# hila-chefer/Transformer-Explainability

Measured on NVIDIA H100. Metric: explanations_per_sec, higher is better.
Workload: dtype f32

## Files before the change

### transformer_explainability_b200/csrc/te_tc_wgmma.cu

```cuda
#include <cuda.h>
#include <cuda_bf16.h>
#include <cuda_fp16.h>
#include <cuda_runtime.h>
#include <string.h>
#include <algorithm>
#include <string>
#include <type_traits>
#include <utility>

#include "te_gemm_tc.h"
#include "te_wgmma.cuh"

namespace {

constexpr int BM = 128, NTHREADS = 256;

__device__ __forceinline__ uint32_t smem_u32(const void* p) { return (uint32_t)__cvta_generic_to_shared(p); }
__device__ __forceinline__ void fence_proxy_async() { asm volatile("fence.proxy.async.shared::cta;" ::: "memory"); }
__device__ __forceinline__ void wg_fence() { asm volatile("wgmma.fence.sync.aligned;" ::: "memory"); }
__device__ __forceinline__ void wg_commit() { asm volatile("wgmma.commit_group.sync.aligned;" ::: "memory"); }
__device__ __forceinline__ void wg_wait0() { asm volatile("wgmma.wait_group.sync.aligned 0;" ::: "memory"); }
__device__ __forceinline__ void wg_wait1() { asm volatile("wgmma.wait_group.sync.aligned 1;" ::: "memory"); }

__device__ __forceinline__ void mbar_init(uint32_t bar, uint32_t count) {
// ... 157 lines not shown
        for (int u = 0; u < 4; ++u) {
            const int k = 4 * c + u;
            e[u] = *reinterpret_cast<const float*>(box + k * 128 + (((m >> 2) ^ (k & 7)) << 4));
        }
        f(r, c, make_float4(e[0], e[1], e[2], e[3]));
    }
}
template <bool SP>
__device__ __forceinline__ auto put_tf32(uint8_t* hi, uint8_t* lo) {
    return [=](int r, int c, float4 v) {
        if (SP) st4(hi, r, c, tf32x4(v));
        else st_split(hi, lo, r, c, v);
    };
}
template <bool SP>
__device__ __forceinline__ void fix_tf32(uint8_t* hi, uint8_t* lo, int r0, int n, int t, int nt) {
    if (SP) map_rows(hi, r0, n, t, nt, [](float4 v) { return tf32x4(v); });
    else split_rows(hi, lo, r0, n, t, nt);
}

__device__ __forceinline__ int frag_row(int tid, int j) { return 64 * (tid >> 7) + 16 * ((tid >> 5) & 3) + ((tid & 31) >> 2) + 8 * ((j >> 1) & 1); }
__device__ __forceinline__ int frag_col(int tid, int j) { return 8 * (j >> 2) + 2 * (tid & 3) + (j & 1); }

struct TmaArgs {
    CUtensorMap map[4];
    int mtiles, ntiles, nz;
};
enum { FIX_NONE = 0, FIX_A = 1, FIX_AB = 2 };
constexpr int NTHREADS_TMA = 384, SMEM_MAX = 227 * 1024;
__host__ __device__ constexpr int tma_stages(int bytes) { return (SMEM_MAX - 1024 - 128) / bytes < 8 ? (SMEM_MAX - 1024 - 128) / bytes : 8; }

template <class P, int NA, int NR, int NT, int NTR>
__device__ __forceinline__ void fold(const P& p, float (&acc)[NA][NR], float (&tot)[NT][NTR], int m0, int ch, int z, int tid) {
    const float s0 = p.chunk_scale(m0 + frag_row(tid, 0), ch, z), s1 = p.chunk_scale(m0 + frag_row(tid, 2), ch, z);
#pragma unroll
    for (int a = 0; a < NA; ++a)
#pragma unroll
        for (int j = 0; j < NR; ++j) tot[a][j] = fmaf(acc[a][j], ((j >> 1) & 1) ? s1 : s0, tot[a][j]);
}
template <int NA, int NR>
__device__ __forceinline__ void zero(float (&v)[NA][NR]) {
#pragma unroll
    for (int a = 0; a < NA; ++a)
#pragma unroll
        for (int j = 0; j < NR; ++j) v[a][j] = 0.f;
}

template <class P>
__device__ __forceinline__ void reg_tile(const P& p, uint8_t* smem, int col_fast) {
    constexpr int NR = P::BN / 2;
    constexpr int NA = P::PRODS::NACC;
    constexpr int STAGE = P::L::BYTES;
    constexpr int NT = P::CHUNK ? NA : 1, NTR = P::CHUNK ? NR : 1;
// ... 1 lines not shown
    const int m0 = (col_fast ? blockIdx.y : blockIdx.x) * BM, n0 = (col_fast ? blockIdx.x : blockIdx.y) * P::BN;
    const int z = blockIdx.z;
    float acc[NA][NR];
    float tot[NT][NTR];
    zero(acc);
    zero(tot);

    const int kb = p.kblocks();
    p.load(smem, 0, m0, n0, z, tid);
    fence_proxy_async();
    __syncthreads();
    for (int it = 0; it < kb; ++it) {
        const bool fresh = P::CHUNK ? (it % P::CHUNK == 0) : (it == 0);
        wg_fence();
        issue<P>(smem_u32(smem + (it & 1) * STAGE), wg, acc, fresh ? 0u : 1u);
        wg_commit();
        if (it + 1 < kb) p.load(smem + ((it + 1) & 1) * STAGE, it + 1, m0, n0, z, tid);
        wg_wait0();
        if constexpr (P::CHUNK > 0)
            if ((it + 1) % P::CHUNK == 0 || it + 1 == kb) fold(p, acc, tot, m0, it / P::CHUNK, z, tid);
        fence_proxy_async();
        __syncthreads();
    }
    if constexpr (P::CHUNK > 0) p.epilogue(tot, m0, n0, z, tid);
    else p.epilogue(acc, m0, n0, z, tid);
}

template <class P>
__device__ __forceinline__ void tma_tiles(const P& p, const TmaArgs& ta, uint8_t* smem) {
    using L = typename P::L;
    constexpr int NR = P::BN / 2;
    constexpr int NA = P::PRODS::NACC;
    constexpr int STAGE = L::BYTES, S = tma_stages(STAGE);
    constexpr int NT = P::CHUNK ? NA : 1, NTR = P::CHUNK ? NR : 1;
    static_assert(S >= 2, "a TMA problem needs two stages");
    __shared__ __align__(8) uint64_t bars[2 * S];
    const int tid = threadIdx.x, wg = tid >> 7;
    const uint32_t full0 = smem_u32(bars), empty0 = full0 + 8u * S, st0 = smem_u32(smem);
    if (tid == 0) {
        for (int s = 0; s < S; ++s) {
            mbar_init(full0 + 8u * s, 1);
            mbar_init(empty0 + 8u * s, 8);
        }
        asm volatile("fence.mbarrier_init.release.cluster;" ::: "memory");
    }
    __syncthreads();
    const int kb = p.kblocks(), per_z = ta.mtiles * ta.ntiles, ntiles = ta.nz * per_z;
    int stage = 0;
    uint32_t phase = 0;
    auto decode = [&](int t, int& m0, int& n0, int& z) {
        z = t / per_z;
        const int r = t - z * per_z;
        m0 = (r / ta.ntiles) * BM;
        n0 = (r % ta.ntiles) * P::BN;
    };

    if (wg == 2) {
        setmaxnreg_dec<40>();
        if (tid != 2 * 128) return;
        for (int t = blockIdx.x; t < ntiles; t += gridDim.x) {
            int m0, n0, z;
            decode(t, m0, n0, z);
            for (int it = 0; it < kb; ++it) {
                mbar_wait(empty0 + 8u * stage, phase ^ 1u);
                p.produce(ta, st0 + (uint32_t)stage * STAGE, full0 + 8u * stage, it, m0, n0, z);
                if (++stage == S) { stage = 0; phase ^= 1u; }
            }
        }
        return;
    }

    setmaxnreg_inc<232>();
    float acc[NA][NR];
    float tot[NT][NTR];
    auto release = [&](int s) {
        if ((tid & 31) == 0) mbar_arrive(empty0 + 8u * s);
    };
    for (int t = blockIdx.x; t < ntiles; t += gridDim.x) {
        int m0, n0, z;
        decode(t, m0, n0, z);
        zero(acc);
        zero(tot);
        int pend = -1;
        for (int it = 0; it < kb; ++it) {
            mbar_wait(full0 + 8u * stage, phase);
            const uint32_t st = st0 + (uint32_t)stage * STAGE;
            if constexpr (P::FIX != FIX_NONE) {
                p.fix(smem + (uint32_t)stage * STAGE, wg, tid);
                fence_proxy_async();
                if constexpr (P::FIX == FIX_A) bar_named(1 + wg, 128);
                else bar_named(3, 256);
            }
            const bool fresh = P::CHUNK ? (it % P::CHUNK == 0) : (it == 0);
            wg_fence();
            issue<P>(st, wg, acc, fresh ? 0u : 1u);
            wg_commit();
            const bool last = it + 1 == kb;
            if (last || (P::CHUNK ? (it + 1) % P::CHUNK == 0 : false)) {
                wg_wait0();
                if (pend >= 0) release(pend);
                release(stage);
                pend = -1;
                if constexpr (P::CHUNK > 0) fold(p, acc, tot, m0, it / P::CHUNK, z, tid);
            } else {
                wg_wait1();
                if (pend >= 0) release(pend);
                pend = stage;
            }
            if (++stage == S) { stage = 0; phase ^= 1u; }
        }
        if constexpr (P::CHUNK > 0) p.epilogue(tot, m0, n0, z, tid);
        else p.epilogue(acc, m0, n0, z, tid);
    }
}

template <class P>
__global__ void __launch_bounds__(P::TMA ? NTHREADS_TMA : NTHREADS, 1)
    wg_kernel(const P p, const __grid_constant__ TmaArgs ta, int col_fast) {
    extern __shared__ uint8_t smem_raw[];
    uint8_t* smem = smem_raw + ((1024u - (smem_u32(smem_raw) & 1023u)) & 1023u);
    if constexpr (P::TMA) tma_tiles(p, ta, smem);
    else reg_tile(p, smem, col_fast);
}

struct NoScale {
    __device__ __forceinline__ float chunk_scale(int, int, int) const { return 1.f; }
};

struct TmaTile {
    const void* base;
    long long rows, cols, ld;
    int box_rows;
    long long count = 0, cstride = 0;
};
template <class P>
// ... 1 lines not shown
    using L = typename P::L;
    constexpr int KE = P::FMT == OP_TF32 ? 32 : 64;
    mbar_expect_tx(bar, L::BYTES);
#pragma unroll
    for (int i = 0; i < L::NTA; ++i) tma_load(st + L::a(i), &ta.map[i], it * KE, m0, bar);
#pragma unroll
    for (int j = 0; j < L::NTB; ++j) tma_load(st + L::b(j), &ta.map[L::NTA + j], it * KE, n0, bar);
}
#define TE_PRODUCE_TILES(P)                                                                                      \
    static constexpr int NMAPS = L::NTA + L::NTB;                                                                \
    __device__ void produce(const TmaArgs& ta, uint32_t st, uint32_t bar, int it, int m0, int n0, int) const { \
        produce_tiles<P>(ta, st, bar, it, m0, n0);                                                               \
    }

enum { ZO_F32 = 0, ZO_BF16 = 1, ZO_F16S = 2 };
template <bool SINGLE, bool BF, int OUT>
struct ZsProb : NoScale {
    static constexpr int BN = 128, CHUNK = 0, FMT = BF ? OP_BF16 : OP_TF32;
    using PRODS = std::conditional_t<SINGLE, One, Prods<Pr<0, 0, 0>, Pr<0, 1, 1>>>;
    using L = Stage<PRODS, BN>;
    static constexpr bool COL_FAST = true;
    static constexpr bool TMA = SINGLE;
    static constexpr int FIX = SINGLE && !BF ? FIX_A : FIX_NONE;
    int M, N, K;
    const float* x; long long ldx;
    const void* xabs;
    const void* wa; const void* wb;
    const float* r; long long ldr; const float* y; long long ldy; const float* bias;
    void* out; long long ldo; float* hs;
    float sscale, zsign;

    __device__ int kblocks() const { return K / (BF ? 64 : 32); }
    __device__ void fix(uint8_t* st, int wg, int tid) const {
        map_rows(st + L::a(0), 64 * wg, 64, tid & 127, 128, [](float4 v) { return tf32x4(absx4(v)); });
    }
    TE_PRODUCE_TILES(ZsProb)
    TmaTile tile(int i) const {
        if (i == 0) return BF ? TmaTile{xabs, M, K, K, BM} : TmaTile{x, M, K, ldx, BM};
        return TmaTile{wa, N, K, K, BN};
    }
    __device__ void load(uint8_t* st, int kb, int m0, int n0, int, int tid) const {
        for_k32(BM, x, ldx, m0, M, kb * 32, K, tid, [&](int rr, int c, float4 v) {
            st4(st + L::a(0), rr, c, tf32x4(posx4(v)));
            st4(st + L::a(1), rr, c, tf32x4(negx4(v)));
        });
        for_k32(BN, (const float*)wa, K, n0, N, kb * 32, K, tid, [&](int rr, int c, float4 v) { st4(st + L::b(0), rr, c, v); });
        for_k32(BN, (const float*)wb, K, n0, N, kb * 32, K, tid, [&](int rr, int c, float4 v) { st4(st + L::b(1), rr, c, v); });
    }
    __device__ void epilogue(float (&acc)[1][BN / 2], int m0, int n0, int, int tid) const {
        float sv[BN / 2];
        float rmax[2] = {0.f, 0.f};
#pragma unroll
        for (int j = 0; j < BN / 2; j += 2) {
            const int row = m0 + frag_row(tid, j), col = n0 + frag_col(tid, j);
            float2 rr = make_float2(0.f, 0.f), z = make_float2(acc[0][j], acc[0][j + 1]);
            if (row < M) {
                rr = *reinterpret_cast<const float2*>(r + (long long)row * ldr + col);
                if (SINGLE) {
                    const float2 yy = *reinterpret_cast<const float2*>(y + (long long)row * ldy + col);
                    const float2 bb = bias ? *reinterpret_cast<const float2*>(bias + col) : make_float2(0.f, 0.f);
                    z.x = 0.5f * ((yy.x - bb.x) + zsign * z.x);
                    z.y = 0.5f * ((yy.y - bb.y) + zsign * z.y);
                    z = zsign > 0.f ? make_float2(fmaxf(z.x, 0.f), fmaxf(z.y, 0.f)) : make_float2(fminf(z.x, 0.f), fminf(z.y, 0.f));
                }
            }
            sv[j] = sscale * te_sd(rr.x, z.x);
            sv[j + 1] = sscale * te_sd(rr.y, z.y);
            if (OUT == ZO_F16S) rmax[(j >> 1) & 1] = fmaxf(rmax[(j >> 1) & 1], fmaxf(fabsf(sv[j]), fabsf(sv[j + 1])));
            if (row >= M) continue;
            if (OUT == ZO_F32) {
                *reinterpret_cast<float2*>((float*)out + (long long)row * ldo + col) = make_float2(to_tf32(sv[j]), to_tf32(sv[j + 1]));
            } else if (OUT == ZO_BF16) {
                *reinterpret_cast<__nv_bfloat162*>((__nv_bfloat16*)out + (long long)row * ldo + col) = __floats2bfloat162_rn(sv[j], sv[j + 1]);
            }
        }
        if (OUT == ZO_F16S) {
            float sc[2];
#pragma unroll
            for (int h = 0; h < 2; ++h) {
                float m = rmax[h];
                m = fmaxf(m, __shfl_xor_sync(0xffffffffu, m, 1));
                m = fmaxf(m, __shfl_xor_sync(0xffffffffu, m, 2));
                float si;
                te_f16_block_scale(m, sc[h], si);
                const int row = m0 + frag_row(tid, 2 * h);
                if ((tid & 3) == 0 && row < M) hs[(long long)row * (N / 128) + n0 / 128] = si;
            }
#pragma unroll
            for (int j = 0; j < BN / 2; j += 2) {
                const int row = m0 + frag_row(tid, j), col = n0 + frag_col(tid, j);
                const float s = sc[(j >> 1) & 1];
                if (row < M) *reinterpret_cast<__half2*>((__half*)out + (long long)row * N + col) = __floats2half2_rn(sv[j] * s, sv[j + 1] * s);
            }
        }
    }
};

template <int KIND>
struct ZrProb {
    static constexpr int BN = (KIND == 2) ? 64 : 128, CHUNK = (KIND == 2) ? 2 : 0;
    static constexpr int FMT = KIND == 0 ? OP_TF32 : KIND == 1 ? OP_BF16 : OP_F16;
    using PRODS = Prods<Pr<0, 0, 0>, Pr<1, 0, 1>>;
    using L = Stage<PRODS, BN>;
    static constexpr bool TMA = true;
    static constexpr int FIX = FIX_NONE;
    int M, N, K;
    const void* s; const void* wp; const void* wn;
    const float* rs; int rs_ld; const float* cp; const float* cn;
    const float* x; long long ldx; float* out; long long ldo;
    int accum;

    __device__ int kblocks() const { return K / (KIND ? 64 : 32); }
    TE_PRODUCE_TILES(ZrProb)
    __device__ float chunk_scale(int row, int ch, int) const { return (KIND == 2 && row < M) ? rs[(long long)row * rs_ld + ch] : 1.f; }
    TmaTile tile(int i) const { return i == 0 ? TmaTile{s, M, K, K, BM} : TmaTile{i == 1 ? wp : wn, N, K, K, BN}; }
    __device__ void epilogue(float (&acc)[2][BN / 2], int m0, int n0, int, int tid) const {
#pragma unroll
        for (int j = 0; j < BN / 2; j += 2) {
            const int row = m0 + frag_row(tid, j), col = n0 + frag_col(tid, j);
            if (row >= M) continue;
            const float2 xv = *reinterpret_cast<const float2*>(x + (long long)row * ldx + col);
            float2 ap = make_float2(acc[0][j], acc[0][j + 1]), an = make_float2(acc[1][j], acc[1][j + 1]);
            if (KIND == 2) {
                ap.x *= cp[col]; ap.y *= cp[col + 1];
                an.x *= cn[col]; an.y *= cn[col + 1];
            }
            float2* o = reinterpret_cast<float2*>(out + (long long)row * ldo + col);
            float2 v = make_float2(fmaxf(xv.x, 0.f) * ap.x + fminf(xv.x, 0.f) * an.x, fmaxf(xv.y, 0.f) * ap.y + fminf(xv.y, 0.f) * an.y);
            if (accum) {
                const float2 prev = *o;
                v = make_float2(prev.x + v.x, prev.y + v.y);
            }
            *o = v;
        }
    }
};

template <bool NEG>
struct LrpSProb : NoScale {
    static constexpr int BN = 128, CHUNK = 0, FMT = OP_TF32;
    using PRODS = One;
    using L = Stage<PRODS, BN>;
    static constexpr bool COL_FAST = true, TMA = false;
    int M, N, K;
    const float* x; long long ldx; const float* w;
    const float* r; long long ldr; float* out;
    float sscale;
    __device__ int kblocks() const { return K / 32; }
    __device__ void load(uint8_t* st, int kb, int m0, int n0, int, int tid) const {
        for_k32(BM, x, ldx, m0, M, kb * 32, K, tid, [&](int rr, int c, float4 v) { st4(st + L::a(0), rr, c, tf32x4(NEG ? negx4(v) : posx4(v))); });
        for_k32(BN, w, K, n0, N, kb * 32, K, tid, [&](int rr, int c, float4 v) { st4(st + L::b(0), rr, c, v); });
    }
    __device__ void epilogue(float (&acc)[1][BN / 2], int m0, int n0, int, int tid) const {
#pragma unroll
        for (int j = 0; j < BN / 2; j += 2) {
            const int row = m0 + frag_row(tid, j), col = n0 + frag_col(tid, j);
            if (row >= M) continue;
            const float2 rr = *reinterpret_cast<const float2*>(r + (long long)row * ldr + col);
            *reinterpret_cast<float2*>(out + (long long)row * N + col) =
                make_float2(to_tf32(sscale * te_sd(rr.x, acc[0][j])), to_tf32(sscale * te_sd(rr.y, acc[0][j + 1])));
        }
    }
};
template <bool NEG>
struct LrpRProb : NoScale {
    static constexpr int BN = 128, CHUNK = 0, FMT = OP_TF32;
    using PRODS = One;
    using L = Stage<PRODS, BN>;
    static constexpr bool TMA = true;
    static constexpr int FIX = FIX_NONE;
    int M, N, K;
    const float* s; const float* wt;
    const float* x; long long ldx; float* out; long long ldo;
    int accum;
    __device__ int kblocks() const { return K / 32; }
    TE_PRODUCE_TILES(LrpRProb)
    TmaTile tile(int i) const { return i == 0 ? TmaTile{s, M, K, K, BM} : TmaTile{wt, N, K, K, BN}; }
    __device__ void epilogue(float (&acc)[1][BN / 2], int m0, int n0, int, int tid) const {
#pragma unroll
        for (int j = 0; j < BN / 2; j += 2) {
            const int row = m0 + frag_row(tid, j), col = n0 + frag_col(tid, j);
            if (row >= M) continue;
            const float2 xv = *reinterpret_cast<const float2*>(x + (long long)row * ldx + col);
            float2* o = reinterpret_cast<float2*>(out + (long long)row * ldo + col);
            if (NEG) {
                const float2 prev = *o;
                *o = make_float2(prev.x + fminf(xv.x, 0.f) * acc[0][j], prev.y + fminf(xv.y, 0.f) * acc[0][j + 1]);
            } else if (accum) {
                const float2 prev = *o;
                *o = make_float2(prev.x + fmaxf(xv.x, 0.f) * acc[0][j], prev.y + fmaxf(xv.y, 0.f) * acc[0][j + 1]);
            } else {
                *o = make_float2(fmaxf(xv.x, 0.f) * acc[0][j], fmaxf(xv.y, 0.f) * acc[0][j + 1]);
            }
        }
    }
};

struct LinOut {
    int M, N;
    const float* bias; const float* E; long long lde;
    float* C; long long ldc; float* C2; long long ldc2;
};
template <int EPI, bool FAST_GRAD = false>
__device__ __forceinline__ void lin_store(const LinOut& o, int row, int col, float v0, float v1) {
    if (row >= o.M) return;
    float2 b = make_float2(0.f, 0.f);
    if ((EPI == TE_TC_EPI_BIAS || EPI == TE_TC_EPI_BIAS_GELU || EPI == TE_TC_EPI_BIAS_ADD) && o.bias)
        b = *reinterpret_cast<const float2*>(o.bias + col);
    float2 y = make_float2(v0 + b.x, v1 + b.y), y2 = make_float2(0.f, 0.f);
    if (EPI == TE_TC_EPI_BIAS_GELU) y2 = make_float2(te_gelu(y.x), te_gelu(y.y));
    if (EPI == TE_TC_EPI_BIAS_ADD || EPI == TE_TC_EPI_GELU_BWD) {
        const float2 e = *reinterpret_cast<const float2*>(o.E + (long long)row * o.lde + col);
        if (EPI == TE_TC_EPI_BIAS_ADD) y2 = make_float2(e.x + y.x, e.y + y.y);
        else if (FAST_GRAD) y = make_float2(v0 * te_gelu_grad_fast(e.x), v1 * te_gelu_grad_fast(e.y));
        else y = make_float2(v0 * te_gelu_grad(e.x), v1 * te_gelu_grad(e.y));
    }
    *reinterpret_cast<float2*>(o.C + (long long)row * o.ldc + col) = y;
    if (EPI == TE_TC_EPI_BIAS_GELU || EPI == TE_TC_EPI_BIAS_ADD) *reinterpret_cast<float2*>(o.C2 + (long long)row * o.ldc2 + col) = y2;
}

enum { LIN_3XTF32 = 0, LIN_TF32 = 1, LIN_F16X3 = 2, LIN_F16 = 3 };
struct LinArgs {
    int K, rs_ld;
    const void* a; const void* a_lo; long long lda;
    const void* b; const void* b_lo;
    const float* rs; const float* cs;
    LinOut o;
};
static_assert(sizeof(LinArgs) <= 128, "LinArgs: keep the kernel parameter within 128 bytes");
template <int EPI, int FORM>
struct LinProb : LinArgs {
    static constexpr bool F16 = FORM == LIN_F16X3 || FORM == LIN_F16, SPLIT = FORM == LIN_3XTF32 || FORM == LIN_F16X3;
    static constexpr int BN = 128, CHUNK = F16 ? 2 : SPLIT ? 4 : 0, FMT = F16 ? OP_F16 : OP_TF32;
    using PRODS = std::conditional_t<SPLIT, Split3, One>;
    using L = Stage<PRODS, BN>;
    static constexpr bool COL_FAST = true;
    static constexpr bool TMA = FORM != LIN_3XTF32;
    static constexpr int FIX = FORM == LIN_TF32 ? FIX_A : FIX_NONE;
    __device__ int kblocks() const { return K / (F16 ? 64 : 32); }
    __device__ float chunk_scale(int row, int ch, int) const {
        if constexpr (F16) return row < o.M ? rs[(long long)row * rs_ld + ch] : 1.f;
        else return 1.f;
    }
    __device__ void fix(uint8_t* st, int wg, int tid) const {
        map_rows(st + L::a(0), 64 * wg, 64, tid & 127, 128, [](float4 v) { return tf32x4(v); });
    }
    TE_PRODUCE_TILES(LinProb)
    TmaTile tile(int i) const {
        if (i < L::NTA) return TmaTile{i == 0 ? a : a_lo, o.M, K, F16 ? K : lda, BM};
        return TmaTile{i == L::NTA ? b : b_lo, o.N, K, K, BN};
    }
    __device__ void load(uint8_t* st, int kb, int m0, int n0, int, int tid) const {
        for_k32(BM, (const float*)a, lda, m0, o.M, kb * 32, K, tid, [&](int r, int c, float4 v) { st_split(st + L::a(0), st + L::a(1), r, c, v); });
        for_k32(BN, (const float*)b, K, n0, o.N, kb * 32, K, tid, [&](int r, int c, float4 v) { st4(st + L::b(0), r, c, v); });
        for_k32(BN, (const float*)b_lo, K, n0, o.N, kb * 32, K, tid, [&](int r, int c, float4 v) { st4(st + L::b(1), r, c, v); });
    }
    __device__ void epilogue(float (&acc)[1][BN / 2], int m0, int n0, int, int tid) const {
#pragma unroll
        for (int j = 0; j < BN / 2; j += 2) {
            const int col = n0 + frag_col(tid, j);
            if constexpr (F16)
                lin_store<EPI>(o, m0 + frag_row(tid, j), col, acc[0][j] * cs[col], acc[0][j + 1] * cs[col + 1]);
            else lin_store<EPI, FORM == LIN_TF32>(o, m0 + frag_row(tid, j), col, acc[0][j], acc[0][j + 1]);
        }
    }
};

enum { AT_STORE = 0, AT_MUL = 1, AT_SD = 2, AT_SOFTMAX = 3, AT_RESID = 4 };
template <int EPI, bool SP, int BN_>
struct NnProb : NoScale {
    static constexpr int BN = BN_, CHUNK = 0, FMT = OP_TF32;
    using PRODS = std::conditional_t<SP, One, Split3>;
    using L = Stage<PRODS, BN>;
    static constexpr bool TMA = true;
    static constexpr int FIX = FIX_AB;
    int N, H, dh, ld_out, batch;
    const float* a; long long lda; const float* b; long long ldb;
    const float* E; float* out; float alpha;
    __device__ int kblocks() const { return dh / 32; }
    static constexpr int NMAPS = 2;
    TmaTile tile(int i) const {
        return i == 0 ? TmaTile{a, (long long)batch * N, H * dh, lda, BM} : TmaTile{b, (long long)batch * N, H * dh, ldb, BN};
    }
    __device__ void produce(const TmaArgs& ta, uint32_t st, uint32_t bar, int kb, int m0, int n0, int bh) const {
        const int s = bh / H, k = (bh % H) * dh + kb * 32;
        mbar_expect_tx(bar, TILE128 + BN * 128);
        tma_load(st + L::a(0), &ta.map[0], k, s * N + m0, bar);
        tma_load(st + L::b(0), &ta.map[1], k, s * N + n0, bar);
    }
    __device__ void fix(uint8_t* st, int wg, int tid) const {
        fix_tf32<SP>(st + L::a(0), st + L::a(1), 64 * wg, 64, tid & 127, 128);
        fix_tf32<SP>(st + L::b(0), st + L::b(1), 0, BN, tid, 256);
    }
    __device__ void epilogue(float (&acc)[1][BN / 2], int m0, int n0, int bh, int tid) const {
        const int ncols = (N + 3) & ~3;
        if constexpr (EPI == AT_SOFTMAX) {
            float mx[2] = {-INFINITY, -INFINITY};
#pragma unroll
            for (int j = 0; j < BN / 2; ++j)
                if (n0 + frag_col(tid, j) < N) mx[(j >> 1) & 1] = fmaxf(mx[(j >> 1) & 1], alpha * acc[0][j]);
            float sum[2] = {0.f, 0.f}, m2[2];
#pragma unroll
            for (int h = 0; h < 2; ++h) {
                mx[h] = fmaxf(mx[h], __shfl_xor_sync(0xffffffffu, mx[h], 1));
                mx[h] = fmaxf(mx[h], __shfl_xor_sync(0xffffffffu, mx[h], 2));
                m2[h] = -mx[h] * 1.4426950408889634f;
            }
            const float a2 = alpha * 1.4426950408889634f;
#pragma unroll
            for (int j = 0; j < BN / 2; ++j) {
                const float e = (n0 + frag_col(tid, j) < N) ? ex2_approx(fmaf(a2, acc[0][j], m2[(j >> 1) & 1])) : 0.f;
                acc[0][j] = e;
                sum[(j >> 1) & 1] += e;
            }
#pragma unroll
            for (int h = 0; h < 2; ++h) {
                sum[h] += __shfl_xor_sync(0xffffffffu, sum[h], 1);
// ... 22 lines not shown
            const long long off = ((long long)bh * N + r) * ld_out + col;
            const float2 e = ef[j / 2];
            float v[2] = {alpha * acc[0][j], alpha * acc[0][j + 1]};
            const float ee[2] = {e.x, e.y};
#pragma unroll
            for (int u = 0; u < 2; ++u) {
                if (EPI == AT_MUL) v[u] *= ee[u];
                else if (EPI == AT_SD) v[u] = te_sd_fast(ee[u], v[u]);
                if (col + u >= N) v[u] = 0.f;
            }
            *reinterpret_cast<float2*>(out + off) = make_float2(v[0], v[1]);
        }
        }
    }
};

template <int AMN, int EPI, bool SP, int BN_>
struct NkProb : NoScale {
    static constexpr int BN = BN_, CHUNK = SP ? 0 : 4, FMT = OP_TF32;
    using PRODS = std::conditional_t<SP, One, Split3>;
    static constexpr int LAND_A = AMN ? BM * 128 : 0, LAND_X = BN * 128;
    using L = Stage<PRODS, BN, LAND_A + LAND_X>;
    static constexpr bool TMA = true;
    static constexpr int FIX = FIX_AB;
    int N, H, NP, ld_out, n_out, n_pad, a_shared, batch;
    const float* map; const float* X; long long ldx;
    const float* rowscale; const float* E; float* out; float alpha;
    __device__ int kblocks() const { return (N + 31) / 32; }
    static constexpr int NMAPS = 2;
    TmaTile tile(int i) const {
        if (i == 0) return TmaTile{map, N, N, NP, AMN ? 32 : BM, (long long)batch * (a_shared ? 1 : H), (long long)N * NP};
        return TmaTile{X, N, n_pad, ldx, 32, batch, (long long)N * ldx};
    }
    __device__ void produce(const TmaArgs& ta, uint32_t st, uint32_t bar, int kb, int m0, int, int bh) const {
        const int s = bh / H, h = bh % H, za = a_shared ? s : bh;
        mbar_expect_tx(bar, (AMN ? LAND_A : TILE128) + LAND_X);
        if (AMN == 0) tma_load3(st + L::a(0), &ta.map[0], kb * 32, m0, za, bar);
#pragma unroll
        for (int j = 0; j < LAND_A / 4096; ++j) tma_load3(st + L::land() + j * 4096, &ta.map[0], m0 + 32 * j, kb * 32, za, bar);
#pragma unroll
        for (int j = 0; j < LAND_X / 4096; ++j)
            tma_load3(st + L::land() + LAND_A + j * 4096, &ta.map[1], h * BN + 32 * j, kb * 32, s, bar);
    }
    __device__ void fix(uint8_t* st, int wg, int tid) const {
        if (AMN) transpose_rows(st + L::land(), 64 * wg, 64, tid & 127, 128, put_tf32<SP>(st + L::a(0), st + L::a(1)));
        else fix_tf32<SP>(st + L::a(0), st + L::a(1), 64 * wg, 64, tid & 127, 128);
        transpose_rows(st + L::land() + LAND_A, 0, BN, tid, 256, put_tf32<SP>(st + L::b(0), st + L::b(1)));
    }
    __device__ void epilogue(float (&acc)[1][BN / 2], int m0, int, int bh, int tid) const {
        const int s = bh / H, h = bh % H;
        float2 ef[BN / 4];
#pragma unroll
        for (int j = 0; j < BN / 2; j += 2) {
            const int m = m0 + frag_row(tid, j), gcol = h * BN + frag_col(tid, j);
            ef[j / 2] = (EPI != AT_STORE && m < N && gcol < n_pad)
                            ? *reinterpret_cast<const float2*>(E + ((long long)s * N + m) * ld_out + gcol) : make_float2(0.f, 0.f);
        }
#pragma unroll
        for (int j = 0; j < BN / 2; j += 2) {
            const int m = m0 + frag_row(tid, j), gcol = h * BN + frag_col(tid, j);
            if (m >= N || gcol >= n_pad) continue;
            const long long off = ((long long)s * N + m) * ld_out + gcol;
            float v[2] = {alpha * acc[0][j], alpha * acc[0][j + 1]};
            const float2 e = ef[j / 2];
            if (EPI == AT_MUL) {
                v[0] *= e.x; v[1] *= e.y;
            } else if (EPI == AT_RESID) {
                const float rsc = rowscale ? rowscale[(long long)s * N + m] : 1.f;
                v[0] += rsc * e.x; v[1] += rsc * e.y;
            }
            if (gcol >= n_out) v[0] = 0.f;
            if (gcol + 1 >= n_out) v[1] = 0.f;
// ... 27 lines not shown
    }();
    return fn;
}
bool encode_tile(CUtensorMap* map, const TmaTile& t, int esize) {
    const EncodeTiled fn = encode_tiled();
    const int rank = t.count > 0 ? 3 : 2;
    if (!fn || ((uintptr_t)t.base & 15u) || (t.ld * esize) % 16 != 0 || (t.cstride * esize) % 16 != 0 || t.rows < 1 || t.cols < 1)
        return false;
    const cuuint64_t dims[3] = {(cuuint64_t)t.cols, (cuuint64_t)t.rows, (cuuint64_t)t.count};
    const cuuint64_t strides[2] = {(cuuint64_t)(t.ld * esize), (cuuint64_t)(t.cstride * esize)};
    const cuuint32_t box[3] = {(cuuint32_t)(128 / esize), (cuuint32_t)t.box_rows, 1}, estr[3] = {1, 1, 1};
    return fn(map, esize == 4 ? CU_TENSOR_MAP_DATA_TYPE_FLOAT32 : CU_TENSOR_MAP_DATA_TYPE_UINT16, rank, const_cast<void*>(t.base),
              dims, strides, box, estr, CU_TENSOR_MAP_INTERLEAVE_NONE, CU_TENSOR_MAP_SWIZZLE_128B,
              CU_TENSOR_MAP_L2_PROMOTION_L2_256B, CU_TENSOR_MAP_FLOAT_OOB_FILL_NONE) == CUDA_SUCCESS;
}

template <class P>
int launch(const P& p, dim3 grid, cudaStream_t st) {
    TmaArgs ta;
    memset(&ta, 0, sizeof(ta));
    int col_fast = 0, threads = NTHREADS, smem = 2 * P::L::BYTES + 1024;
    if constexpr (P::TMA) {
        constexpr int ESIZE = P::FMT == OP_TF32 ? 4 : 2;
        static_assert(P::NMAPS <= 4, "TmaArgs holds four tensor maps");
        for (int i = 0; i < P::NMAPS; ++i)
            if (!encode_tile(&ta.map[i], p.tile(i), ESIZE)) {
                te_set_last_error("te_tc: cannot encode a TMA tensor map (16-byte-aligned base and strides required)");
                return TE_ERR_ARG;
            }
        const long long tiles = (long long)grid.x * grid.y * grid.z;
        if (tiles > INT32_MAX) { te_set_last_error("te_tc: grid too large for one launch"); return TE_ERR_ARG; }
        ta.mtiles = (int)grid.x;
        ta.ntiles = (int)grid.y;
        ta.nz = (int)grid.z;
        grid = dim3((unsigned)std::min<long long>(tiles, sm_count()));
        threads = NTHREADS_TMA;
        smem = tma_stages(P::L::BYTES) * P::L::BYTES + 1024;
    } else {
        col_fast = P::COL_FAST && grid.x <= 65535;
        if (col_fast) grid = dim3(grid.y, grid.x, grid.z);
    }
    static unsigned long long done = 0;
    int dev = 0;
    if (cudaGetDevice(&dev) != cudaSuccess) { te_set_last_error("te_tc: cudaGetDevice failed"); return TE_ERR_CUDA; }
    if (!(done & (1ull << (dev & 63)))) {
        if (cudaFuncSetAttribute(wg_kernel<P>, cudaFuncAttributeMaxDynamicSharedMemorySize, smem) != cudaSuccess) {
            te_set_last_error("te_tc: cannot raise dynamic shared memory");
            return TE_ERR_CUDA;
        }
        done |= 1ull << (dev & 63);
    }
    if (grid.y > 65535 || grid.z > 65535) { te_set_last_error("te_tc: grid too large for one launch"); return TE_ERR_ARG; }
    wg_kernel<P><<<grid, threads, smem, st>>>(p, ta, col_fast);
    TE_CUDA_CHECK_LAUNCH();
    return TE_OK;
}
inline unsigned mtiles(long long M) { return (unsigned)((M + BM - 1) / BM); }

__global__ void prepare_weights_kernel(const float* __restrict__ w, float* __restrict__ d, int out_f, int in_f) {
    const TeDerived<float> dv(d, in_f, out_f);
// ... 169 lines not shown
    return TE_OK;
}

int te_tc_blocksplit_f16(const float* x, long long ldx, long long rows, int cols, float* split, float* scale_inv, cudaStream_t st,
                         bool hi_only) {
    if (cols % 4 != 0 || ldx % 4 != 0 || !a16(x) || !a16(split) || !scale_inv) {
        te_set_last_error("te_tc_blocksplit_f16: alignment");
        return TE_ERR_ARG;
    }
    __half* hi = reinterpret_cast<__half*>(split);
    blocksplit_f16_kernel<<<stride_blocks(rows, 8), 256, 0, st>>>(x, ldx, rows, cols, hi, hi_only ? nullptr : hi + rows * cols,
                                                                  scale_inv);
    TE_CUDA_CHECK_LAUNCH();
    return TE_OK;
}

bool te_tc_zplus_supported(long long rows, int in_features, int out_features, long long ldx) {
    return rows > 0 && rows < (1LL << 31) && in_features % 128 == 0 && out_features % 128 == 0 && ldx % 4 == 0;
}
int te_tc_zplus_s1(const float* x, long long ldx, float* xabs, const float* derived, const float* r, long long ldr,
                   const float* y, long long ldy, const float* bias, float* s_out, long long rows, int in_features,
                   int out_features, cudaStream_t st, bool bf16, float* s16, float* s16_scale, float s_scale, bool inh) {
    const TeDerived<const float> dv(derived, in_features, out_features);
    if (ldx % 4 != 0 || !a16(x) || !a16(r) || !a16(y) || ldr % 2 != 0 || ldy % 2 != 0) {
        te_set_last_error("te_tc_zplus_s1: alignment");
        return TE_ERR_ARG;
    }
    void* o = s16 ? (void*)s16 : (void*)s_out;
    auto run = [&](auto zs_fn, const void* wa) {
        return zs_fn(x, ldx, xabs, wa, nullptr, r, ldr, y, ldy, bias, o, s16_scale, rows, in_features, out_features, st, s_scale,
                     inh);
    };
    if (bf16 && in_features % 64 == 0) {
        if (!a16(xabs)) { te_set_last_error("te_tc_zplus_s1: alignment"); return TE_ERR_ARG; }
        abs_bf16_kernel<<<stride_blocks(rows * (in_features / 4), 256), 256, 0, st>>>(
            x, ldx, reinterpret_cast<__nv_bfloat16*>(xabs), rows, in_features / 4);
        TE_CUDA_CHECK_LAUNCH();
        return s16 ? run(zs<true, true, ZO_F16S>, dv.bf_wabs) : run(zs<true, true, ZO_F32>, dv.bf_wabs);
    }
    return s16 ? run(zs<true, false, ZO_F16S>, dv.wabs) : run(zs<true, false, ZO_F32>, dv.wabs);
}

int te_tc_zplus_r(const float* s, const float* derived, const float* x, long long ldx, float* out, long long ld_out,
                  long long rows, int in_features, int out_features, cudaStream_t st, bool inh) {
    const TeDerived<const float> dv(derived, in_features, out_features);
    ZrProb<0> p;
    memset(&p, 0, sizeof(p));
// ... 247 lines not shown
```

Baseline: 796.5.

## Prefetch epilogue operand tiles via TMA into shared memory during mainloop

Adds extra TMA tensor maps for the epilogue operands (r/y, x, E) and has the producer warp load them into a dedicated shared-memory buffer once the first stages are issued. The epilogue then reads these tiles from swizzled shared memory instead of doing scattered global float2 loads, and it is split into a compute pass and a store pass. The consumer loop is also restructured into per-chunk blocks. This hides epilogue global-load latency behind the mainloop, at the cost of fewer pipeline stages because the epilogue buffer takes shared memory, plus a single-buffered epilogue barrier that can serialize consecutive tiles.

```diff
diff --git a/transformer_explainability_b200/csrc/te_tc_wgmma.cu b/transformer_explainability_b200/csrc/te_tc_wgmma.cu
--- a/transformer_explainability_b200/csrc/te_tc_wgmma.cu
+++ b/transformer_explainability_b200/csrc/te_tc_wgmma.cu
@@ -203,13 +203,22 @@
 __device__ __forceinline__ int frag_row(int tid, int j) { return 64 * (tid >> 7) + 16 * ((tid >> 5) & 3) + ((tid & 31) >> 2) + 8 * ((j >> 1) & 1); }
 __device__ __forceinline__ int frag_col(int tid, int j) { return 8 * (j >> 2) + 2 * (tid & 3) + (j & 1); }
 
+constexpr int TMA_MAPS = 5;
 struct TmaArgs {
-    CUtensorMap map[4];
+    CUtensorMap map[TMA_MAPS];
     int mtiles, ntiles, nz;
 };
 enum { FIX_NONE = 0, FIX_A = 1, FIX_AB = 2 };
 constexpr int NTHREADS_TMA = 384, SMEM_MAX = 227 * 1024;
-__host__ __device__ constexpr int tma_stages(int bytes) { return (SMEM_MAX - 1024 - 128) / bytes < 8 ? (SMEM_MAX - 1024 - 128) / bytes : 8; }
+__host__ __device__ constexpr int tma_stages(int bytes, int epi) {
+    return (SMEM_MAX - 1024 - 256 - epi) / bytes < 8 ? (SMEM_MAX - 1024 - 256 - epi) / bytes : 8;
+}
+
+template <class P>
+__host__ __device__ constexpr int epi_bytes() { return P::EPI_MAPS * BM * P::BN * 4; }
+__device__ __forceinline__ float2 epi_f2(const uint8_t* t, int r, int c) {
+    return *reinterpret_cast<const float2*>(t + (c >> 5) * (BM * 128) + swz(r, (c & 31) >> 2) + (c & 3) * 4);
+}
 
 template <class P, int NA, int NR, int NT, int NTR>
 __device__ __forceinline__ void fold(const P& p, float (&acc)[NA][NR], float (&tot)[NT][NTR], int m0, int ch, int z, int tid) {
@@ -257,8 +266,8 @@
         fence_proxy_async();
         __syncthreads();
     }
-    if constexpr (P::CHUNK > 0) p.epilogue(tot, m0, n0, z, tid);
-    else p.epilogue(acc, m0, n0, z, tid);
+    if constexpr (P::CHUNK > 0) p.epilogue(tot, m0, n0, z, tid, nullptr);
+    else p.epilogue(acc, m0, n0, z, tid, nullptr);
 }
 
 template <class P>
@@ -266,17 +275,20 @@
     using L = typename P::L;
     constexpr int NR = P::BN / 2;
     constexpr int NA = P::PRODS::NACC;
-    constexpr int STAGE = L::BYTES, S = tma_stages(STAGE);
+    constexpr int STAGE = L::BYTES, EPI = epi_bytes<P>(), S = tma_stages(STAGE, EPI);
     constexpr int NT = P::CHUNK ? NA : 1, NTR = P::CHUNK ? NR : 1;
     static_assert(S >= 2, "a TMA problem needs two stages");
-    __shared__ __align__(8) uint64_t bars[2 * S];
+    __shared__ __align__(8) uint64_t bars[2 * S + 2];
     const int tid = threadIdx.x, wg = tid >> 7;
     const uint32_t full0 = smem_u32(bars), empty0 = full0 + 8u * S, st0 = smem_u32(smem);
+    const uint32_t efull = full0 + 16u * S, eempty = efull + 8u, ebuf = st0 + (uint32_t)S * STAGE;
     if (tid == 0) {
         for (int s = 0; s < S; ++s) {
             mbar_init(full0 + 8u * s, 1);
             mbar_init(empty0 + 8u * s, 8);
         }
+        mbar_init(efull, 1);
+        mbar_init(eempty, 8);
         asm volatile("fence.mbarrier_init.release.cluster;" ::: "memory");
     }
     __syncthreads();
@@ -293,6 +305,7 @@
     if (wg == 2) {
         setmaxnreg_dec<40>();
         if (tid != 2 * 128) return;
+        uint32_t ephase = 0;
         for (int t = blockIdx.x; t < ntiles; t += gridDim.x) {
             int m0, n0, z;
             decode(t, m0, n0, z);
@@ -300,6 +313,19 @@
                 mbar_wait(empty0 + 8u * stage, phase ^ 1u);
                 p.produce(ta, st0 + (uint32_t)stage * STAGE, full0 + 8u * stage, it, m0, n0, z);
                 if (++stage == S) { stage = 0; phase ^= 1u; }
+                if constexpr (EPI > 0) {
+                    if (it == min(S, kb) - 1) {
+                        mbar_wait(eempty, ephase ^ 1u);
+                        mbar_expect_tx(efull, EPI);
+#pragma unroll
+                        for (int i = 0; i < P::EPI_MAPS; ++i)
+#pragma unroll
+                            for (int b = 0; b < P::BN / 32; ++b)
+                                tma_load(ebuf + (uint32_t)(i * BM * P::BN * 4 + b * BM * 128), &ta.map[P::NMAPS + i], n0 + 32 * b,
+                                         m0, efull);
+                        ephase ^= 1u;
+                    }
+                }
             }
         }
         return;
@@ -311,41 +337,51 @@
     auto release = [&](int s) {
         if ((tid & 31) == 0) mbar_arrive(empty0 + 8u * s);
     };
+    auto consume = [&](uint32_t sd) {
+        mbar_wait(full0 + 8u * stage, phase);
+        if constexpr (P::FIX != FIX_NONE) {
+            p.fix(smem + (uint32_t)stage * STAGE, wg, tid);
+            fence_proxy_async();
+            if constexpr (P::FIX == FIX_A) bar_named(1 + wg, 128);
+            else bar_named(3, 256);
+        }
+        wg_fence();
+        issue<P>(st0 + (uint32_t)stage * STAGE, wg, acc, sd);
+        wg_commit();
+    };
+    auto next = [&] {
+        if (++stage == S) { stage = 0; phase ^= 1u; }
+    };
+    constexpr int CH = P::CHUNK;
+    uint32_t ephase = 0;
     for (int t = blockIdx.x; t < ntiles; t += gridDim.x) {
         int m0, n0, z;
         decode(t, m0, n0, z);
         zero(acc);
         zero(tot);
-        int pend = -1;
-        for (int it = 0; it < kb; ++it) {
-            mbar_wait(full0 + 8u * stage, phase);
-            const uint32_t st = st0 + (uint32_t)stage * STAGE;
-            if constexpr (P::FIX != FIX_NONE) {
-                p.fix(smem + (uint32_t)stage * STAGE, wg, tid);
-                fence_proxy_async();
-                if constexpr (P::FIX == FIX_A) bar_named(1 + wg, 128);
-                else bar_named(3, 256);
-            }
-            const bool fresh = P::CHUNK ? (it % P::CHUNK == 0) : (it == 0);
-            wg_fence();
-            issue<P>(st, wg, acc, fresh ? 0u : 1u);
-            wg_commit();
-            const bool last = it + 1 == kb;
-            if (last || (P::CHUNK ? (it + 1) % P::CHUNK == 0 : false)) {
-                wg_wait0();
-                if (pend >= 0) release(pend);
-                release(stage);
-                pend = -1;
-                if constexpr (P::CHUNK > 0) fold(p, acc, tot, m0, it / P::CHUNK, z, tid);
-            } else {
+        for (int k0 = 0; k0 < kb; k0 += CH ? CH : kb) {
+            const int k1 = CH ? min(k0 + CH, kb) : kb;
+            consume(0u);
+            for (int it = k0 + 1; it < k1; ++it) {
+                const int prev = stage;
+                next();
+                consume(1u);
                 wg_wait1();
-                if (pend >= 0) release(pend);
-                pend = stage;
-            }
-            if (++stage == S) { stage = 0; phase ^= 1u; }
-        }
-        if constexpr (P::CHUNK > 0) p.epilogue(tot, m0, n0, z, tid);
-        else p.epilogue(acc, m0, n0, z, tid);
+                release(prev);
+            }
+            wg_wait0();
+            release(stage);
+            next();
+            if constexpr (CH > 0) fold(p, acc, tot, m0, k0 / CH, z, tid);
+        }
+        if constexpr (EPI > 0) mbar_wait(efull, ephase);
+        if constexpr (P::CHUNK > 0) p.epilogue(tot, m0, n0, z, tid, smem + (uint32_t)S * STAGE);
+        else p.epilogue(acc, m0, n0, z, tid, smem + (uint32_t)S * STAGE);
+        if constexpr (EPI > 0) {
+            __syncwarp();
+            if ((tid & 31) == 0) mbar_arrive(eempty);
+            ephase ^= 1u;
+        }
     }
 }
 
@@ -393,6 +429,7 @@
     static constexpr bool COL_FAST = true;
     static constexpr bool TMA = SINGLE;
     static constexpr int FIX = SINGLE && !BF ? FIX_A : FIX_NONE;
+    static constexpr int EPI_MAPS = SINGLE ? 2 : 0;
     int M, N, K;
     const float* x; long long ldx;
     const void* xabs;
@@ -408,7 +445,8 @@
     TE_PRODUCE_TILES(ZsProb)
     TmaTile tile(int i) const {
         if (i == 0) return BF ? TmaTile{xabs, M, K, K, BM} : TmaTile{x, M, K, ldx, BM};
-        return TmaTile{wa, N, K, K, BN};
+        if (i == 1) return TmaTile{wa, N, K, K, BN};
+        return i == 2 ? TmaTile{r, M, N, ldr, BM} : TmaTile{y, M, N, ldy, BM};
     }
     __device__ void load(uint8_t* st, int kb, int m0, int n0, int, int tid) const {
         for_k32(BM, x, ldx, m0, M, kb * 32, K, tid, [&](int rr, int c, float4 v) {
@@ -418,7 +456,7 @@
         for_k32(BN, (const float*)wa, K, n0, N, kb * 32, K, tid, [&](int rr, int c, float4 v) { st4(st + L::b(0), rr, c, v); });
         for_k32(BN, (const float*)wb, K, n0, N, kb * 32, K, tid, [&](int rr, int c, float4 v) { st4(st + L::b(1), rr, c, v); });
     }
-    __device__ void epilogue(float (&acc)[1][BN / 2], int m0, int n0, int, int tid) const {
+    __device__ void epilogue(float (&acc)[1][BN / 2], int m0, int n0, int, int tid, const uint8_t* eb) const {
         float sv[BN / 2];
         float rmax[2] = {0.f, 0.f};
 #pragma unroll
@@ -426,9 +464,10 @@
             const int row = m0 + frag_row(tid, j), col = n0 + frag_col(tid, j);
             float2 rr = make_float2(0.f, 0.f), z = make_float2(acc[0][j], acc[0][j + 1]);
             if (row < M) {
-                rr = *reinterpret_cast<const float2*>(r + (long long)row * ldr + col);
+                rr = SINGLE ? epi_f2(eb, frag_row(tid, j), frag_col(tid, j))
+                            : *reinterpret_cast<const float2*>(r + (long long)row * ldr + col);
                 if (SINGLE) {
-                    const float2 yy = *reinterpret_cast<const float2*>(y + (long long)row * ldy + col);
+                    const float2 yy = epi_f2(eb + BM * BN * 4, frag_row(tid, j), frag_col(tid, j));
                     const float2 bb = bias ? *reinterpret_cast<const float2*>(bias + col) : make_float2(0.f, 0.f);
                     z.x = 0.5f * ((yy.x - bb.x) + zsign * z.x);
                     z.y = 0.5f * ((yy.y - bb.y) + zsign * z.y);
@@ -438,6 +477,10 @@
             sv[j] = sscale * te_sd(rr.x, z.x);
             sv[j + 1] = sscale * te_sd(rr.y, z.y);
             if (OUT == ZO_F16S) rmax[(j >> 1) & 1] = fmaxf(rmax[(j >> 1) & 1], fmaxf(fabsf(sv[j]), fabsf(sv[j + 1])));
+        }
+#pragma unroll
+        for (int j = 0; j < BN / 2; j += 2) {
+            const int row = m0 + frag_row(tid, j), col = n0 + frag_col(tid, j);
             if (row >= M) continue;
             if (OUT == ZO_F32) {
                 *reinterpret_cast<float2*>((float*)out + (long long)row * ldo + col) = make_float2(to_tf32(sv[j]), to_tf32(sv[j + 1]));
@@ -474,7 +517,7 @@
     using PRODS = Prods<Pr<0, 0, 0>, Pr<1, 0, 1>>;
     using L = Stage<PRODS, BN>;
     static constexpr bool TMA = true;
-    static constexpr int FIX = FIX_NONE;
+    static constexpr int FIX = FIX_NONE, EPI_MAPS = 1;
     int M, N, K;
     const void* s; const void* wp; const void* wn;
     const float* rs; int rs_ld; const float* cp; const float* cn;
@@ -484,25 +527,33 @@
     __device__ int kblocks() const { return K / (KIND ? 64 : 32); }
     TE_PRODUCE_TILES(ZrProb)
     __device__ float chunk_scale(int row, int ch, int) const { return (KIND == 2 && row < M) ? rs[(long long)row * rs_ld + ch] : 1.f; }
-    TmaTile tile(int i) const { return i == 0 ? TmaTile{s, M, K, K, BM} : TmaTile{i == 1 ? wp : wn, N, K, K, BN}; }
-    __device__ void epilogue(float (&acc)[2][BN / 2], int m0, int n0, int, int tid) const {
+    TmaTile tile(int i) const {
+        if (i == 0) return TmaTile{s, M, K, K, BM};
+        return i < 3 ? TmaTile{i == 1 ? wp : wn, N, K, K, BN} : TmaTile{x, M, N, ldx, BM};
+    }
+    __device__ void epilogue(float (&acc)[2][BN / 2], int m0, int n0, int, int tid, const uint8_t* eb) const {
 #pragma unroll
         for (int j = 0; j < BN / 2; j += 2) {
             const int row = m0 + frag_row(tid, j), col = n0 + frag_col(tid, j);
             if (row >= M) continue;
-            const float2 xv = *reinterpret_cast<const float2*>(x + (long long)row * ldx + col);
+            const float2 xv = epi_f2(eb, frag_row(tid, j), frag_col(tid, j));
             float2 ap = make_float2(acc[0][j], acc[0][j + 1]), an = make_float2(acc[1][j], acc[1][j + 1]);
             if (KIND == 2) {
                 ap.x *= cp[col]; ap.y *= cp[col + 1];
                 an.x *= cn[col]; an.y *= cn[col + 1];
             }
-            float2* o = reinterpret_cast<float2*>(out + (long long)row * ldo + col);
             float2 v = make_float2(fmaxf(xv.x, 0.f) * ap.x + fminf(xv.x, 0.f) * an.x, fmaxf(xv.y, 0.f) * ap.y + fminf(xv.y, 0.f) * an.y);
             if (accum) {
-                const float2 prev = *o;
+                const float2 prev = *reinterpret_cast<const float2*>(out + (long long)row * ldo + col);
                 v = make_float2(prev.x + v.x, prev.y + v.y);
             }
-            *o = v;
+            acc[0][j] = v.x;
+            acc[0][j + 1] = v.y;
+        }
+#pragma unroll
+        for (int j = 0; j < BN / 2; j += 2) {
+            const int row = m0 + frag_row(tid, j), col = n0 + frag_col(tid, j);
+            if (row < M) *reinterpret_cast<float2*>(out + (long long)row * ldo + col) = make_float2(acc[0][j], acc[0][j + 1]);
         }
     }
 };
@@ -522,7 +573,7 @@
         for_k32(BM, x, ldx, m0, M, kb * 32, K, tid, [&](int rr, int c, float4 v) { st4(st + L::a(0), rr, c, tf32x4(NEG ? negx4(v) : posx4(v))); });
         for_k32(BN, w, K, n0, N, kb * 32, K, tid, [&](int rr, int c, float4 v) { st4(st + L::b(0), rr, c, v); });
     }
-    __device__ void epilogue(float (&acc)[1][BN / 2], int m0, int n0, int, int tid) const {
+    __device__ void epilogue(float (&acc)[1][BN / 2], int m0, int n0, int, int tid, const uint8_t*) const {
 #pragma unroll
         for (int j = 0; j < BN / 2; j += 2) {
             const int row = m0 + frag_row(tid, j), col = n0 + frag_col(tid, j);
@@ -539,30 +590,40 @@
     using PRODS = One;
     using L = Stage<PRODS, BN>;
     static constexpr bool TMA = true;
-    static constexpr int FIX = FIX_NONE;
+    static constexpr int FIX = FIX_NONE, EPI_MAPS = 1;
     int M, N, K;
     const float* s; const float* wt;
     const float* x; long long ldx; float* out; long long ldo;
     int accum;
     __device__ int kblocks() const { return K / 32; }
     TE_PRODUCE_TILES(LrpRProb)
-    TmaTile tile(int i) const { return i == 0 ? TmaTile{s, M, K, K, BM} : TmaTile{wt, N, K, K, BN}; }
-    __device__ void epilogue(float (&acc)[1][BN / 2], int m0, int n0, int, int tid) const {
+    TmaTile tile(int i) const {
+        return i == 0 ? TmaTile{s, M, K, K, BM} : i == 1 ? TmaTile{wt, N, K, K, BN} : TmaTile{x, M, N, ldx, BM};
+    }
+    __device__ void epilogue(float (&acc)[1][BN / 2], int m0, int n0, int, int tid, const uint8_t* eb) const {
 #pragma unroll
         for (int j = 0; j < BN / 2; j += 2) {
             const int row = m0 + frag_row(tid, j), col = n0 + frag_col(tid, j);
             if (row >= M) continue;
-            const float2 xv = *reinterpret_cast<const float2*>(x + (long long)row * ldx + col);
-            float2* o = reinterpret_cast<float2*>(out + (long long)row * ldo + col);
+            const float2 xv = epi_f2(eb, frag_row(tid, j), frag_col(tid, j));
+            const float2* o = reinterpret_cast<const float2*>(out + (long long)row * ldo + col);
+            float2 v;
             if (NEG) {
                 const float2 prev = *o;
-                *o = make_float2(prev.x + fminf(xv.x, 0.f) * acc[0][j], prev.y + fminf(xv.y, 0.f) * acc[0][j + 1]);
+                v = make_float2(prev.x + fminf(xv.x, 0.f) * acc[0][j], prev.y + fminf(xv.y, 0.f) * acc[0][j + 1]);
             } else if (accum) {
                 const float2 prev = *o;
-                *o = make_float2(prev.x + fmaxf(xv.x, 0.f) * acc[0][j], prev.y + fmaxf(xv.y, 0.f) * acc[0][j + 1]);
+                v = make_float2(prev.x + fmaxf(xv.x, 0.f) * acc[0][j], prev.y + fmaxf(xv.y, 0.f) * acc[0][j + 1]);
             } else {
-                *o = make_float2(fmaxf(xv.x, 0.f) * acc[0][j], fmaxf(xv.y, 0.f) * acc[0][j + 1]);
-            }
+                v = make_float2(fmaxf(xv.x, 0.f) * acc[0][j], fmaxf(xv.y, 0.f) * acc[0][j + 1]);
+            }
+            acc[0][j] = v.x;
+            acc[0][j + 1] = v.y;
+        }
+#pragma unroll
+        for (int j = 0; j < BN / 2; j += 2) {
+            const int row = m0 + frag_row(tid, j), col = n0 + frag_col(tid, j);
+            if (row < M) *reinterpret_cast<float2*>(out + (long long)row * ldo + col) = make_float2(acc[0][j], acc[0][j + 1]);
         }
     }
 };
@@ -572,21 +633,27 @@
     const float* bias; const float* E; long long lde;
     float* C; long long ldc; float* C2; long long ldc2;
 };
-template <int EPI, bool FAST_GRAD = false>
-__device__ __forceinline__ void lin_store(const LinOut& o, int row, int col, float v0, float v1) {
-    if (row >= o.M) return;
+template <int EPI, bool FAST_GRAD, class EF>
+__device__ __forceinline__ float2 lin_value(const LinOut& o, int col, float v0, float v1, EF e) {
     float2 b = make_float2(0.f, 0.f);
     if ((EPI == TE_TC_EPI_BIAS || EPI == TE_TC_EPI_BIAS_GELU || EPI == TE_TC_EPI_BIAS_ADD) && o.bias)
         b = *reinterpret_cast<const float2*>(o.bias + col);
-    float2 y = make_float2(v0 + b.x, v1 + b.y), y2 = make_float2(0.f, 0.f);
+    if (EPI == TE_TC_EPI_GELU_BWD) {
+        const float2 ev = e();
+        if (FAST_GRAD) return make_float2(v0 * te_gelu_grad_fast(ev.x), v1 * te_gelu_grad_fast(ev.y));
+        return make_float2(v0 * te_gelu_grad(ev.x), v1 * te_gelu_grad(ev.y));
+    }
+    return make_float2(v0 + b.x, v1 + b.y);
+}
+template <int EPI, class EF>
+__device__ __forceinline__ void lin_store(const LinOut& o, int row, int col, float2 y, EF e) {
+    *reinterpret_cast<float2*>(o.C + (long long)row * o.ldc + col) = y;
+    float2 y2 = make_float2(0.f, 0.f);
     if (EPI == TE_TC_EPI_BIAS_GELU) y2 = make_float2(te_gelu(y.x), te_gelu(y.y));
-    if (EPI == TE_TC_EPI_BIAS_ADD || EPI == TE_TC_EPI_GELU_BWD) {
-        const float2 e = *reinterpret_cast<const float2*>(o.E + (long long)row * o.lde + col);
-        if (EPI == TE_TC_EPI_BIAS_ADD) y2 = make_float2(e.x + y.x, e.y + y.y);
-        else if (FAST_GRAD) y = make_float2(v0 * te_gelu_grad_fast(e.x), v1 * te_gelu_grad_fast(e.y));
-        else y = make_float2(v0 * te_gelu_grad(e.x), v1 * te_gelu_grad(e.y));
-    }
-    *reinterpret_cast<float2*>(o.C + (long long)row * o.ldc + col) = y;
+    if (EPI == TE_TC_EPI_BIAS_ADD) {
+        const float2 ev = e();
+        y2 = make_float2(ev.x + y.x, ev.y + y.y);
+    }
     if (EPI == TE_TC_EPI_BIAS_GELU || EPI == TE_TC_EPI_BIAS_ADD) *reinterpret_cast<float2*>(o.C2 + (long long)row * o.ldc2 + col) = y2;
 }
 
@@ -608,6 +675,7 @@
     static constexpr bool COL_FAST = true;
     static constexpr bool TMA = FORM != LIN_3XTF32;
     static constexpr int FIX = FORM == LIN_TF32 ? FIX_A : FIX_NONE;
+    static constexpr int EPI_MAPS = TMA && (EPI == TE_TC_EPI_BIAS_ADD || EPI == TE_TC_EPI_GELU_BWD) ? 1 : 0;
     __device__ int kblocks() const { return K / (F16 ? 64 : 32); }
     __device__ float chunk_scale(int row, int ch, int) const {
         if constexpr (F16) return row < o.M ? rs[(long long)row * rs_ld + ch] : 1.f;
@@ -619,21 +687,36 @@
     TE_PRODUCE_TILES(LinProb)
     TmaTile tile(int i) const {
         if (i < L::NTA) return TmaTile{i == 0 ? a : a_lo, o.M, K, F16 ? K : lda, BM};
-        return TmaTile{i == L::NTA ? b : b_lo, o.N, K, K, BN};
+        if (i < NMAPS) return TmaTile{i == L::NTA ? b : b_lo, o.N, K, K, BN};
+        return TmaTile{o.E, o.M, o.N, o.lde, BM};
     }
     __device__ void load(uint8_t* st, int kb, int m0, int n0, int, int tid) const {
         for_k32(BM, (const float*)a, lda, m0, o.M, kb * 32, K, tid, [&](int r, int c, float4 v) { st_split(st + L::a(0), st + L::a(1), r, c, v); });
         for_k32(BN, (const float*)b, K, n0, o.N, kb * 32, K, tid, [&](int r, int c, float4 v) { st4(st + L::b(0), r, c, v); });
         for_k32(BN, (const float*)b_lo, K, n0, o.N, kb * 32, K, tid, [&](int r, int c, float4 v) { st4(st + L::b(1), r, c, v); });
     }
-    __device__ void epilogue(float (&acc)[1][BN / 2], int m0, int n0, int, int tid) const {
+    __device__ void epilogue(float (&acc)[1][BN / 2], int m0, int n0, int, int tid, const uint8_t* eb) const {
 #pragma unroll
         for (int j = 0; j < BN / 2; j += 2) {
-            const int col = n0 + frag_col(tid, j);
+            const int row = m0 + frag_row(tid, j), col = n0 + frag_col(tid, j);
+            if (row >= o.M) continue;
+            auto e = [&] { return efrag(eb, tid, j, row, col); };
+            float2 y;
             if constexpr (F16)
-                lin_store<EPI>(o, m0 + frag_row(tid, j), col, acc[0][j] * cs[col], acc[0][j + 1] * cs[col + 1]);
-            else lin_store<EPI, FORM == LIN_TF32>(o, m0 + frag_row(tid, j), col, acc[0][j], acc[0][j + 1]);
-        }
+                y = lin_value<EPI, false>(o, col, acc[0][j] * cs[col], acc[0][j + 1] * cs[col + 1], e);
+            else y = lin_value<EPI, FORM == LIN_TF32>(o, col, acc[0][j], acc[0][j + 1], e);
+            acc[0][j] = y.x;
+            acc[0][j + 1] = y.y;
+        }
+#pragma unroll
+        for (int j = 0; j < BN / 2; j += 2) {
+            const int row = m0 + frag_row(tid, j), col = n0 + frag_col(tid, j);
+            if (row < o.M) lin_store<EPI>(o, row, col, make_float2(acc[0][j], acc[0][j + 1]), [&] { return efrag(eb, tid, j, row, col); });
+        }
+    }
+    __device__ float2 efrag(const uint8_t* eb, int tid, int j, int row, int col) const {
+        if constexpr (EPI_MAPS > 0) return epi_f2(eb, frag_row(tid, j), frag_col(tid, j));
+        else return *reinterpret_cast<const float2*>(o.E + (long long)row * o.lde + col);
     }
 };
 
@@ -644,7 +727,7 @@
     using PRODS = std::conditional_t<SP, One, Split3>;
     using L = Stage<PRODS, BN>;
     static constexpr bool TMA = true;
-    static constexpr int FIX = FIX_AB;
+    static constexpr int FIX = FIX_AB, EPI_MAPS = 0;
     int N, H, dh, ld_out, batch;
     const float* a; long long lda; const float* b; long long ldb;
     const float* E; float* out; float alpha;
@@ -663,7 +746,7 @@
         fix_tf32<SP>(st + L::a(0), st + L::a(1), 64 * wg, 64, tid & 127, 128);
         fix_tf32<SP>(st + L::b(0), st + L::b(1), 0, BN, tid, 256);
     }
-    __device__ void epilogue(float (&acc)[1][BN / 2], int m0, int n0, int bh, int tid) const {
+    __device__ void epilogue(float (&acc)[1][BN / 2], int m0, int n0, int bh, int tid, const uint8_t*) const {
         const int ncols = (N + 3) & ~3;
         if constexpr (EPI == AT_SOFTMAX) {
             float mx[2] = {-INFINITY, -INFINITY};
@@ -732,7 +815,7 @@
     static constexpr int LAND_A = AMN ? BM * 128 : 0, LAND_X = BN * 128;
     using L = Stage<PRODS, BN, LAND_A + LAND_X>;
     static constexpr bool TMA = true;
-    static constexpr int FIX = FIX_AB;
+    static constexpr int FIX = FIX_AB, EPI_MAPS = 0;
     int N, H, NP, ld_out, n_out, n_pad, a_shared, batch;
     const float* map; const float* X; long long ldx;
     const float* rowscale; const float* E; float* out; float alpha;
@@ -757,7 +840,7 @@
         else fix_tf32<SP>(st + L::a(0), st + L::a(1), 64 * wg, 64, tid & 127, 128);
         transpose_rows(st + L::land() + LAND_A, 0, BN, tid, 256, put_tf32<SP>(st + L::b(0), st + L::b(1)));
     }
-    __device__ void epilogue(float (&acc)[1][BN / 2], int m0, int, int bh, int tid) const {
+    __device__ void epilogue(float (&acc)[1][BN / 2], int m0, int, int bh, int tid, const uint8_t*) const {
         const int s = bh / H, h = bh % H;
         float2 ef[BN / 4];
 #pragma unroll
@@ -831,9 +914,9 @@
     int col_fast = 0, threads = NTHREADS, smem = 2 * P::L::BYTES + 1024;
     if constexpr (P::TMA) {
         constexpr int ESIZE = P::FMT == OP_TF32 ? 4 : 2;
-        static_assert(P::NMAPS <= 4, "TmaArgs holds four tensor maps");
-        for (int i = 0; i < P::NMAPS; ++i)
-            if (!encode_tile(&ta.map[i], p.tile(i), ESIZE)) {
+        static_assert(P::NMAPS + P::EPI_MAPS <= TMA_MAPS, "TmaArgs holds TMA_MAPS tensor maps");
+        for (int i = 0; i < P::NMAPS + P::EPI_MAPS; ++i)
+            if (!encode_tile(&ta.map[i], p.tile(i), i < P::NMAPS ? ESIZE : 4)) {
                 te_set_last_error("te_tc: cannot encode a TMA tensor map (16-byte-aligned base and strides required)");
                 return TE_ERR_ARG;
             }
@@ -844,7 +927,7 @@
         ta.nz = (int)grid.z;
         grid = dim3((unsigned)std::min<long long>(tiles, sm_count()));
         threads = NTHREADS_TMA;
-        smem = tma_stages(P::L::BYTES) * P::L::BYTES + 1024;
+        smem = tma_stages(P::L::BYTES, epi_bytes<P>()) * P::L::BYTES + epi_bytes<P>() + 1024;
     } else {
         col_fast = P::COL_FAST && grid.x <= 65535;
         if (col_fast) grid = dim3(grid.y, grid.x, grid.z);
@@ -1060,7 +1143,7 @@
                    const float* y, long long ldy, const float* bias, float* s_out, long long rows, int in_features,
                    int out_features, cudaStream_t st, bool bf16, float* s16, float* s16_scale, float s_scale, bool inh) {
     const TeDerived<const float> dv(derived, in_features, out_features);
-    if (ldx % 4 != 0 || !a16(x) || !a16(r) || !a16(y) || ldr % 2 != 0 || ldy % 2 != 0) {
+    if (ldx % 4 != 0 || !a16(x) || !a16(r) || !a16(y) || ldr % 4 != 0 || ldy % 4 != 0) {
         te_set_last_error("te_tc_zplus_s1: alignment");
         return TE_ERR_ARG;
     }
```

New measurement: 881.6 (median of 6 runs). 1.11x the previous value.
